# scylladb/vector-store

Measured on NVIDIA B200. Metric: ann_search_qps_at_recall10_ge_0.95, higher is better.
Workload: dtype bf16

## Files before the change

vector-store_b200/csrc/graph_search.cuh:

```cuda
#pragma once
#ifdef VSB_K4B_PROFILE
#include <cstdio>
#endif
#include "kernels.h"
#include "select.cuh"

namespace vsb {

constexpr int K4_WARPS = 4;
constexpr uint32_t kHashEmpty = 0xFFFFFFFFu;

struct K4Args {
    const uint8_t* q_rows;
    const float* q_nrm;
    uint32_t nq, q_row_bytes;
    const uint8_t* x_rows;
    const float* x_nrm;
    uint32_t x_row_bytes;
    const uint32_t* graph;
    uint32_t graph_stride, degree;
    const uint64_t* seed_lists;
    uint32_t seed_splits, n_seeds;
    const uint32_t* seed_slots;
    const uint32_t* deny;
    const uint64_t* keys;
    uint32_t itopk, max_iters, k, hash_bits, search_width, queue_cap;
    int metric;
    uint64_t* out_keys;
    float* out_dists;
    uint32_t* out_counts;
    uint64_t* out_packed;
    long long self_base;
    uint32_t out_stride;
    unsigned long long* counters;
    const uint32_t* allow;
    uint64_t allow_bits;
    uint32_t rk;
    uint32_t mma;
    uint32_t compact;
    uint32_t l2pf;
};

__device__ __forceinline__ bool hash_insert(uint32_t* tab, uint32_t mask, uint32_t bits, uint32_t slot) {
    uint32_t h = (slot * 0x9E3779B1u) >> (32 - bits);
#pragma unroll 1
    for (int probe = 0; probe < 64; ++probe) {
        const uint32_t old = atomicCAS(&tab[h], kHashEmpty, slot);
        if (old == kHashEmpty) return true;
        if (old == slot) return false;
        h = (h + 1) & mask;
    }
    return false;
}

constexpr uint16_t kTagEmpty = 0xFFFFu;
__device__ __forceinline__ bool hash_insert16(uint16_t* tab, uint32_t mask, uint32_t bits, uint32_t slot) {
    uint32_t h = (slot * 0x9E3779B1u) >> (32 - bits);
    uint32_t t = (slot * 0x85EBCA6Bu) >> 16;
    const unsigned short tag = (unsigned short)(t == kTagEmpty ? 0xFFFEu : t);
#pragma unroll 1
    for (int probe = 0; probe < 64; ++probe) {
        const unsigned short old = atomicCAS(reinterpret_cast<unsigned short*>(&tab[h]), (unsigned short)kTagEmpty, tag);
        if (old == kTagEmpty) return true;
        if (old == tag) return false;
        h = (h + 1) & mask;
    }
    return false;
}

template <int CPL, int U>
struct VecGroup {
    uint4 x[U][CPL];
};

template <int CPL, int U>
__device__ __forceinline__ void group_load(VecGroup<CPL, U>& g, const uint8_t* __restrict__ x_rows, uint32_t row_bytes,
                                           const uint32_t* newq, uint32_t base, uint32_t stride, uint32_t last,
                                           int lane, int n_chunks, bool full) {
#pragma unroll
    for (int u = 0; u < U; ++u) {
        uint32_t idx = base + u * stride;
        idx = idx < last ? idx : last;
        const uint4* xrow = reinterpret_cast<const uint4*>(x_rows + (size_t)newq[idx] * row_bytes) + lane;
        if (full) {
#pragma unroll
            for (int j = 0; j < CPL; ++j) g.x[u][j] = ldg_nc_v4(xrow + j * 32);
        } else {
#pragma unroll
            for (int j = 0; j < CPL; ++j) {
                g.x[u][j] = make_uint4(0, 0, 0, 0);
                if (j * 32 + lane < n_chunks) g.x[u][j] = ldg_nc_v4(xrow + j * 32);
            }
        }
    }
}

template <int ST, int CPL, int U>
__device__ __forceinline__ void group_reduce(const VecGroup<CPL, U>& g, const float* qf, const uint4* qc, bool is_l2,
                                             float* newd, uint32_t base, uint32_t stride, uint32_t n_new, int lane) {
    constexpr int E = Storage<ST>::ELEMS;
    constexpr bool kFloat = Storage<ST>::kFloat;
#pragma unroll
    for (int u = 0; u < U; ++u) {
        const uint32_t idx = base + u * stride;
        float raw;
        if constexpr (kFloat) {
            float f;
            if (is_l2) {
                ChunkAcc<ST, VSB_METRIC_L2SQ> acc;
#pragma unroll
                for (int j = 0; j < CPL; ++j) {
                    float xf[E];
                    Storage<ST>::unpack(g.x[u][j], xf);
                    acc.add_f(&qf[j * E], xf);
                }
                f = acc.f;
            } else {
                ChunkAcc<ST, VSB_METRIC_IP> acc;
#pragma unroll
                for (int j = 0; j < CPL; ++j) {
                    float xf[E];
                    Storage<ST>::unpack(g.x[u][j], xf);
                    acc.add_f(&qf[j * E], xf);
                }
                f = acc.f;
            }
            raw = butterfly_sum(f);
        } else {
            int i;
            if (is_l2) {
                ChunkAcc<ST, VSB_METRIC_L2SQ> acc;
#pragma unroll
                for (int j = 0; j < CPL; ++j) acc.add(qc[j], g.x[u][j]);
                i = acc.i;
            } else {
                ChunkAcc<ST, VSB_METRIC_IP> acc;
#pragma unroll
                for (int j = 0; j < CPL; ++j) acc.add(qc[j], g.x[u][j]);
                i = acc.i;
            }
            raw = (float)butterfly_sum_i(i);
        }
        if (lane == 0 && idx < n_new) newd[idx] = raw;
    }
}

template <int ST>
__device__ __forceinline__ float finish_raw(float raw, int metric, float qn, float xn) {
    if constexpr (ST == VSB_ST_B1) {
        return raw;
    } else {
        if (metric == VSB_METRIC_L2SQ) return raw;
        if (metric == VSB_METRIC_IP) {
            if constexpr (ST == VSB_ST_I8) raw = __fdiv_rn(raw, 16129.0f);
            return __fsub_rn(1.0f, raw);
        }
        if (qn == 0.0f && xn == 0.0f) return 0.0f;
        if (qn == 0.0f || xn == 0.0f) return 1.0f;
        float d = __fsub_rn(1.0f, __fdiv_rn(raw, __fmul_rn(qn, xn)));
        d = d < 0.0f ? 0.0f : d;
        d = d > 2.0f ? 2.0f : d;
        return d;
    }
}

template <int ST>
__device__ __forceinline__ void mma_16816(float (&c)[4], uint32_t a0, uint32_t a1, uint32_t a2, uint32_t a3, uint32_t b0,
                                          uint32_t b1) {
    if constexpr (ST == VSB_ST_BF16) {
        asm volatile("mma.sync.aligned.m16n8k16.row.col.f32.bf16.bf16.f32 {%0,%1,%2,%3}, {%4,%5,%6,%7}, {%8,%9}, {%0,%1,%2,%3};"
                     : "+f"(c[0]), "+f"(c[1]), "+f"(c[2]), "+f"(c[3])
                     : "r"(a0), "r"(a1), "r"(a2), "r"(a3), "r"(b0), "r"(b1));
    } else {
        asm volatile("mma.sync.aligned.m16n8k16.row.col.f32.f16.f16.f32 {%0,%1,%2,%3}, {%4,%5,%6,%7}, {%8,%9}, {%0,%1,%2,%3};"
                     : "+f"(c[0]), "+f"(c[1]), "+f"(c[2]), "+f"(c[3])
                     : "r"(a0), "r"(a1), "r"(a2), "r"(a3), "r"(b0), "r"(b1));
    }
}

template <int ST, int CPL, int U>
__device__ __forceinline__ void group_reduce_mma(const VecGroup<CPL, U>& grp, const uint4* qc, float* newd, uint32_t base,
                                                 uint32_t stride, uint32_t n_new, int lane) {
    const int g = lane >> 2, t = lane & 3;
    const bool diag = t == (g >> 1);
    const bool odd = (g & 1) != 0;
#pragma unroll
    for (int u = 0; u < U; u += 2) {
        constexpr bool kPair = U > 1;
        float c[4] = {0.f, 0.f, 0.f, 0.f};
#pragma unroll
        for (int j = 0; j < CPL; ++j) {
            const uint4 xa = grp.x[u][j];
            const uint4 xb = kPair ? grp.x[kPair ? u + 1 : u][j] : xa;
            mma_16816<ST>(c, xa.x, xb.x, xa.y, xb.y, qc[j].x, qc[j].y);
            mma_16816<ST>(c, xa.z, xb.z, xa.w, xb.w, qc[j].z, qc[j].w);
        }
        float v0 = diag ? (odd ? c[1] : c[0]) : 0.0f;
        float v1 = diag ? (odd ? c[3] : c[2]) : 0.0f;
        v0 = butterfly_sum(v0);
        if (kPair) v1 = butterfly_sum(v1);
        if (lane == 0) {
            const uint32_t i0 = base + u * stride, i1 = base + (u + 1) * stride;
            if (i0 < n_new) newd[i0] = v0;
            if (kPair && i1 < n_new) newd[i1] = v1;
        }
    }
}

__device__ __forceinline__ void prefetch_row_l2(const void* p, uint32_t bytes) {
    asm volatile("cp.async.bulk.prefetch.L2.global [%0], %1;" ::"l"(p), "r"(bytes) : "memory");
}

template <int ST, int CPL, int U, bool MMA = false>
__device__ __forceinline__ void evaluate_entries(const uint8_t* __restrict__ x_rows, uint32_t row_bytes,
                                                 const uint32_t* newq, float* newd, uint32_t first, uint32_t stride,
                                                 uint32_t mine, uint32_t n_new, const float* qf, const uint4* qc,
                                                 bool is_l2, int lane, int n_chunks, bool full, uint32_t l2pf = 0) {
    if (mine == 0) return;
    const uint32_t last = first + (mine - 1) * stride;
    if (l2pf != 0) {
        for (uint32_t m = 2 * U + lane; m < l2pf + 2 * U && m < mine; m += 32)
            prefetch_row_l2(x_rows + (size_t)newq[first + m * stride] * row_bytes, row_bytes);
    }
    auto reduce = [&](const VecGroup<CPL, U>& grp, uint32_t base) {
        if constexpr (MMA) group_reduce_mma<ST, CPL, U>(grp, qc, newd, base, stride, n_new, lane);
        else group_reduce<ST, CPL, U>(grp, qf, qc, is_l2, newd, base, stride, n_new, lane);
    };
    VecGroup<CPL, U> ga, gb;
    group_load<CPL, U>(ga, x_rows, row_bytes, newq, first, stride, last, lane, n_chunks, full);
    for (uint32_t m0 = 0; m0 < mine; m0 += 2 * U) {
        const bool has_b = m0 + U < mine;
        if (l2pf != 0) {
            const uint32_t m = m0 + 2 * U + l2pf + lane;
            if (lane < 2 * U && m < mine) prefetch_row_l2(x_rows + (size_t)newq[first + m * stride] * row_bytes, row_bytes);
        }
        if (has_b) group_load<CPL, U>(gb, x_rows, row_bytes, newq, first + (m0 + U) * stride, stride, last, lane, n_chunks, full);
        reduce(ga, first + m0 * stride);
        if (has_b) {
            if (m0 + 2 * U < mine)
                group_load<CPL, U>(ga, x_rows, row_bytes, newq, first + (m0 + 2 * U) * stride, stride, last, lane, n_chunks, full);
            reduce(gb, first + (m0 + U) * stride);
        }
    }
}

#ifndef VSB_K4_MAX_WIDTH
#define VSB_K4_MAX_WIDTH 4
#endif
constexpr int K4_MAX_WIDTH = VSB_K4_MAX_WIDTH;

template <int ST, int CPL, bool MMA = false>
constexpr int k4_min_blocks() { return (ST == VSB_ST_I8 && CPL <= 2) ? 4 : 3; }
template <int CPL, bool MMA>
constexpr int k4_rows_per_group() { return CPL <= 3 ? 4 : (CPL <= 6 ? 2 : 1); }

template <int ST, int CPL, bool FILTER, bool MMA = false>
__global__ void __launch_bounds__(K4_WARPS * 32, k4_min_blocks<ST, CPL, MMA>()) graph_search_kernel(K4Args a) {
    constexpr int E = Storage<ST>::ELEMS;
    constexpr bool kFloat = Storage<ST>::kFloat;
    constexpr int U = k4_rows_per_group<CPL, MMA>();
    constexpr int QF = (kFloat && !MMA) ? CPL * E : 1;

    extern __shared__ __align__(16) uint8_t smem_raw[];
    const int lane = threadIdx.x & 31, warp = threadIdx.x >> 5;
    const uint32_t q = blockIdx.x * K4_WARPS + warp;
    if (q >= a.nq) return;

    const uint32_t hsize = 1u << a.hash_bits, hmask = hsize - 1;
    const uint32_t qcap = a.queue_cap;
    const size_t per_warp = (size_t)a.itopk * 8 + (size_t)hsize * 2 + (size_t)qcap * 8 + (FILTER ? (size_t)a.rk * 8 : 0) + 64 * 8;
    uint64_t* list = reinterpret_cast<uint64_t*>(smem_raw + (size_t)warp * per_warp);
    uint16_t* hash = reinterpret_cast<uint16_t*>(list + a.itopk);
    uint32_t* newq = reinterpret_cast<uint32_t*>(hash + hsize);
    float* newd = reinterpret_cast<float*>(newq + qcap);
    uint64_t* rlist = reinterpret_cast<uint64_t*>(newd + qcap);
    uint64_t* stage = rlist + (FILTER ? a.rk : 0);
    if constexpr (FILTER) {
        for (uint32_t i = lane; i < a.rk; i += 32) rlist[i] = kInvalidPacked;
    }
    const LessBySlot less;
    const bool is_l2 = a.metric == VSB_METRIC_L2SQ;
    const bool is_cos = a.metric == VSB_METRIC_COS;
    const int n_chunks = a.x_row_bytes / 16;
    const bool full = n_chunks == CPL * 32;

    for (uint32_t i = lane; i < a.itopk; i += 32) list[i] = kInvalidPacked;
    for (uint32_t i = lane; i < hsize; i += 32) hash[i] = kTagEmpty;

    const uint4* qrow = reinterpret_cast<const uint4*>(a.q_rows + (size_t)q * a.q_row_bytes);
    float qf[QF];
    uint4 qc[(kFloat && !MMA) ? 1 : CPL];
#pragma unroll
    for (int j = 0; j < CPL; ++j) {
        const int c = j * 32 + lane;
        uint4 v = make_uint4(0, 0, 0, 0);
        if (c < n_chunks) v = qrow[c];
        if constexpr (kFloat && !MMA)
            Storage<ST>::unpack(v, &qf[j * E]);
        else
            qc[j] = v;
    }
    if constexpr (MMA) qf[0] = 0.0f;
    const float qn = a.q_nrm[q];
    __syncwarp();

    uint32_t n_hashed = 0, n_new = 0;
    unsigned long long n_evals = 0, n_parents = 0;

    auto enqueue = [&](uint32_t nb) {
        bool is_new = false;
        if (nb != kInvalidSlot) is_new = hash_insert16(hash, hmask, a.hash_bits, nb);
        const uint32_t m = __ballot_sync(kFullMask, is_new);
        if (is_new) newq[n_new + __popc(m & ((1u << lane) - 1))] = nb;
        n_new += __popc(m);
        n_hashed += __popc(m);
    };

    auto evaluate_queue = [&]() {
        __syncwarp();
        if (n_new == 0) return;
        n_evals += n_new;
        float xn_pre[2] = {0.0f, 0.0f};
        if constexpr (MMA) {
            if (is_cos || is_l2) {
                if (lane < n_new) xn_pre[0] = __ldg(a.x_nrm + newq[lane]);
                if (32 + lane < n_new) xn_pre[1] = __ldg(a.x_nrm + newq[32 + lane]);
            }
        }
        evaluate_entries<ST, CPL, U, MMA>(a.x_rows, a.x_row_bytes, newq, newd, 0, 1, n_new, n_new, qf, qc, is_l2, lane,
                                          n_chunks, full, a.l2pf);
        __syncwarp();
        uint64_t worst = list[a.itopk - 1];
        uint32_t n_stage = 0;
        auto fold_stage = [&](uint32_t n) {
            __syncwarp();
            uint64_t v = lane < n ? stage[lane] : kInvalidPacked;
            v = warp_sort32(v, lane, less);
            warp_list_merge(list, (int)a.itopk, v, lane, less);
            worst = list[a.itopk - 1];
        };
        for (uint32_t base = 0; base < n_new; base += 32) {
            uint64_t res = kInvalidPacked;
            if (base + lane < n_new) {
                const uint32_t slot = newq[base + lane];
                float xn = 0.0f;
                if (MMA && base < 64) xn = base == 0 ? xn_pre[0] : xn_pre[1];
                else if (is_cos || (MMA && is_l2)) xn = __ldg(a.x_nrm + slot);
                float raw = newd[base + lane];
                if constexpr (MMA) {
                    if (is_l2) raw = fmaxf(fmaf(-2.0f, raw, fmaf(qn, qn, xn * xn)), 0.0f);
                }
                res = pack_ds(finish_raw<ST>(raw, a.metric, qn, xn), slot);
            }
            if constexpr (FILTER) {
                uint64_t adm = kInvalidPacked;
                if (res != kInvalidPacked) {
                    const uint64_t row_id = a.keys[packed_lo(res)] & kRowMask48;
                    if (row_id < a.allow_bits && (a.allow[row_id >> 5] >> (row_id & 31) & 1u)) adm = res;
                }
                if (__ballot_sync(kFullMask, adm < rlist[a.rk - 1]) != 0) {
                    adm = warp_sort32(adm, lane, less);
                    warp_list_merge(rlist, (int)a.rk, adm, lane, less);
                }
            }
            const bool keep = res < worst;
            const uint32_t km = __ballot_sync(kFullMask, keep);
            if (km == 0) continue;
            if (!a.compact || n_new <= 32) {
                res = warp_sort32(res, lane, less);
                warp_list_merge(list, (int)a.itopk, res, lane, less);
                continue;
            }
            if (keep) stage[n_stage + __popc(km & ((1u << lane) - 1))] = res;
            n_stage += __popc(km);
            if (n_stage >= 32) {
                fold_stage(32);
                __syncwarp();
                const uint64_t mv = lane + 32 < n_stage ? stage[32 + lane] : kInvalidPacked;
                __syncwarp();
                if (lane + 32 < n_stage) stage[lane] = mv;
                n_stage -= 32;
            }
        }
        if (n_stage != 0) fold_stage(n_stage);
        n_new = 0;
    };

    {
        uint64_t sv = kInvalidPacked;
        for (uint32_t s = 0; s < a.seed_splits; ++s) {
            uint64_t v = a.seed_lists[((size_t)q * a.seed_splits + s) * 32 + lane];
            v = warp_sort32(v, lane, less);
            const uint64_t rc = shfl_u64(v, 31 - lane);
            sv = warp_bitonic_merge32(rc < sv ? rc : sv, lane, less);
        }
        uint32_t nb = kInvalidSlot;
        if (lane < (int)a.n_seeds && sv != kInvalidPacked) nb = a.seed_slots[packed_lo(sv)];
        enqueue(nb);
        evaluate_queue();
    }

    const uint32_t width = a.search_width;
    for (uint32_t it = 0; it < a.max_iters; ++it) {
        if (n_hashed > (hsize >> 2) * 3) {
            for (uint32_t i = lane; i < hsize; i += 32) hash[i] = kTagEmpty;
            __syncwarp();
            n_hashed = 0;
            for (uint32_t b = 0; b < a.itopk; b += 32) {
                const uint64_t e = list[b + lane];
                if (e != kInvalidPacked) hash_insert16(hash, hmask, a.hash_bits, packed_lo(e) & ~kExpandedBit);
                n_hashed += __popc(__ballot_sync(kFullMask, e != kInvalidPacked));
            }
            __syncwarp();
        }
        uint32_t par[K4_MAX_WIDTH];
        uint32_t np = 0;
#pragma unroll
        for (int i = 0; i < K4_MAX_WIDTH; ++i) par[i] = kInvalidSlot;
        for (uint32_t b = 0; b < a.itopk && np < width; b += 32) {
            const uint64_t e = list[b + lane];
            const bool unexp = e != kInvalidPacked && !(packed_lo(e) & kExpandedBit);
            uint32_t m = __ballot_sync(kFullMask, unexp);
            bool mine = false;
            while (m && np < width) {
                const int src = __ffs(m) - 1;
                m &= m - 1;
                const uint32_t pslot = __shfl_sync(kFullMask, packed_lo(e), src);
#pragma unroll
                for (int i = 0; i < K4_MAX_WIDTH; ++i)
                    if (i == (int)np) par[i] = pslot;
                if (lane == src) mine = true;
                ++np;
            }
            if (mine) list[b + lane] = e | kExpandedBit;
        }
        __syncwarp();
        if (np == 0) break;
        n_parents += np;
        uint32_t nbs[K4_MAX_WIDTH][2];
#pragma unroll
        for (int i = 0; i < K4_MAX_WIDTH; ++i) {
#pragma unroll
            for (int h = 0; h < 2; ++h) {
                nbs[i][h] = kInvalidSlot;
                const uint32_t r = h * 32 + lane;
                if (i < (int)np && r < a.degree) nbs[i][h] = __ldg(a.graph + (size_t)par[i] * a.graph_stride + r);
            }
        }
#pragma unroll
        for (int i = 0; i < K4_MAX_WIDTH; ++i) {
#pragma unroll
            for (int h = 0; h < 2; ++h) {
                if (i < (int)np && h * 32 < (int)a.degree) enqueue(nbs[i][h]);
            }
        }
        evaluate_queue();
    }

    __syncwarp();
    const uint64_t* src_list = FILTER ? rlist : list;
    const uint32_t src_len = FILTER ? a.rk : a.itopk;
    uint32_t count = 0;
    for (uint32_t b = 0; b < src_len; b += 32) {
        const uint64_t e = src_list[b + lane];
        const uint32_t slot = packed_lo(e) & ~kExpandedBit;
        bool valid = e != kInvalidPacked;
        if (valid && a.deny != nullptr && bit_test(a.deny, slot)) valid = false;
        if (valid && a.self_base >= 0 && slot == (uint32_t)(a.self_base + q)) valid = false;
        const uint32_t m = __ballot_sync(kFullMask, valid);
        const uint32_t pos = count + __popc(m & ((1u << lane) - 1));
        if (valid && pos < a.k) {
            if (a.out_packed != nullptr) {
                a.out_packed[(size_t)q * a.out_stride + pos] = ((uint64_t)packed_hi(e) << 32) | slot;
            } else {
                a.out_keys[(size_t)q * a.k + pos] = a.keys[slot];
                a.out_dists[(size_t)q * a.k + pos] = ord_to_f32(packed_hi(e));
            }
        }
        count += __popc(m);
    }
    if (count > a.k) count = a.k;
    if (a.out_packed != nullptr) {
        for (uint32_t i = count + lane; i < a.out_stride; i += 32) a.out_packed[(size_t)q * a.out_stride + i] = kInvalidPacked;
    }
    for (uint32_t i = count + lane; i < a.k; i += 32) {
        if (a.out_packed != nullptr) {
        } else {
            a.out_keys[(size_t)q * a.k + i] = 0xFFFFFFFFFFFFFFFFull;
            a.out_dists[(size_t)q * a.k + i] = __int_as_float(0x7F800000);
        }
    }
    if (lane == 0) {
        if (a.out_counts != nullptr) a.out_counts[q] = count;
        if (a.counters != nullptr) {
            atomicAdd(&a.counters[0], n_evals);
            atomicAdd(&a.counters[1], n_parents);
        }
    }
}

constexpr int K4B_WARPS = 8;
constexpr int K4B_MAX_WIDTH = 8;
constexpr int K4B_PICK_ROUNDS = 4;

#ifdef VSB_K4B_PROFILE
#define K4B_T(i)                                       \
    do {                                               \
        const long long now_ = clock64();              \
        prof_[i] += now_ - prof_t_;                    \
        prof_t_ = now_;                                \
    } while (0)
#else
#define K4B_T(i) do { } while (0)
#endif

template <int ST, int CPL>
__global__ void __launch_bounds__(K4B_WARPS * 32, 1) graph_search_cta_kernel(K4Args a) {
    constexpr int E = Storage<ST>::ELEMS;
    constexpr bool kFloat = Storage<ST>::kFloat;
    constexpr int U = CPL <= 3 ? 4 : (CPL <= 6 ? 2 : 1);
    constexpr int QF = kFloat ? CPL * E : 1;

    extern __shared__ __align__(16) uint8_t smem_raw[];
    const int tid = threadIdx.x, lane = tid & 31, warp = tid >> 5;
    const uint32_t q = blockIdx.x;
    const uint32_t hsize = 1u << a.hash_bits, hmask = hsize - 1;
    const uint32_t qcap = a.queue_cap;
    uint64_t* list = reinterpret_cast<uint64_t*>(smem_raw);
    uint64_t* list_alt = list + a.itopk;
    uint64_t* newp = list_alt + a.itopk;
    uint32_t* hash = reinterpret_cast<uint32_t*>(newp + qcap);
    uint32_t* newq = hash + hsize;
    float* newd = reinterpret_cast<float*>(newq + qcap);
    uint32_t* par = reinterpret_cast<uint32_t*>(newd + qcap);
    uint32_t* ctrl = par + K4B_MAX_WIDTH;
    uint32_t* wcnt = ctrl + 4;
    const LessBySlot less;
    const bool is_l2 = a.metric == VSB_METRIC_L2SQ;
    const bool is_cos = a.metric == VSB_METRIC_COS;
    const int n_chunks = a.x_row_bytes / 16;
    const bool full = n_chunks == CPL * 32;

    for (uint32_t i = tid; i < a.itopk; i += K4B_WARPS * 32) list[i] = kInvalidPacked;
    for (uint32_t i = tid; i < hsize; i += K4B_WARPS * 32) hash[i] = kHashEmpty;
    if (tid < 4) ctrl[tid] = 0;

    const uint4* qrow = reinterpret_cast<const uint4*>(a.q_rows + (size_t)q * a.q_row_bytes);
    float qf[QF];
    uint4 qc[kFloat ? 1 : CPL];
#pragma unroll
    for (int j = 0; j < CPL; ++j) {
        const int c = j * 32 + lane;
        uint4 v = make_uint4(0, 0, 0, 0);
        if (c < n_chunks) v = qrow[c];
        if constexpr (kFloat)
            Storage<ST>::unpack(v, &qf[j * E]);
        else
            qc[j] = v;
    }
    const float qn = a.q_nrm[q];
    unsigned long long n_evals = 0, n_parents = 0;
    __syncthreads();
#ifdef VSB_K4B_PROFILE
    long long prof_[8] = {0, 0, 0, 0, 0, 0, 0, 0};
    long long prof_t_ = clock64();
    const long long prof_start_ = prof_t_;
#endif

    const uint32_t width = a.search_width;
    const uint32_t deg_pad = ((a.degree + 31) / 32) * 32;
    auto pick_parents = [&]() {
        uint64_t e[K4B_PICK_ROUNDS];
        uint32_t m[K4B_PICK_ROUNDS];
#pragma unroll
        for (int r = 0; r < K4B_PICK_ROUNDS; ++r) {
            const uint32_t t = r * K4B_WARPS * 32 + tid;
            e[r] = t < a.itopk ? list[t] : kInvalidPacked;
            const bool unexp = e[r] != kInvalidPacked && !(packed_lo(e[r]) & kExpandedBit);
            m[r] = __ballot_sync(kFullMask, unexp);
            if (lane == 0) wcnt[r * K4B_WARPS + warp] = __popc(m[r]);
        }
        __syncthreads();
        uint32_t before = 0, total = 0;
#pragma unroll
        for (int r = 0; r < K4B_PICK_ROUNDS; ++r) {
#pragma unroll
            for (int w = 0; w < K4B_WARPS; ++w) {
                const uint32_t c = wcnt[r * K4B_WARPS + w];
                total += c;
            }
        }
#pragma unroll
        for (int r = 0; r < K4B_PICK_ROUNDS; ++r) {
            uint32_t base = before;
#pragma unroll
            for (int w = 0; w < K4B_WARPS; ++w) {
                const uint32_t c = wcnt[r * K4B_WARPS + w];
                if (w < warp) base += c;
                before += c;
            }
            if (m[r] >> lane & 1u) {
                const uint32_t rank = base + __popc(m[r] & ((1u << lane) - 1));
                if (rank < width) {
                    par[rank] = packed_lo(e[r]);
                    list[r * K4B_WARPS * 32 + tid] = e[r] | kExpandedBit;
                } else if (rank < 2 * width) {
                    asm volatile("prefetch.global.L2 [%0];" ::"l"(a.graph + (size_t)packed_lo(e[r]) * a.graph_stride));
                }
            }
        }
        const uint32_t np = total < width ? total : width;
        if (tid == 0) {
            ctrl[1] = np;
            n_parents += np;
        }
        __syncthreads();
    };

    auto lower_bound = [&](const uint64_t* seq, uint32_t len, uint64_t x) -> uint32_t {
        uint32_t lo = 0, n = len;
        while (n > 0) {
            const uint32_t half = n >> 1;
            const bool go = seq[lo + half] < x;
            lo = go ? lo + half + 1 : lo;
            n = go ? n - half - 1 : half;
        }
        return lo;
    };

    auto evaluate_queue = [&]() {
        K4B_T(0);
        __syncthreads();
        K4B_T(1);
        const uint32_t n_new = ctrl[0];
        if (n_new != 0) {
            const uint32_t mine = n_new > (uint32_t)warp ? (n_new - warp + K4B_WARPS - 1) / K4B_WARPS : 0;
            float xn_first = 0.0f;
            if (is_cos && (uint32_t)tid < n_new) xn_first = __ldg(a.x_nrm + newq[tid]);
            evaluate_entries<ST, CPL, U>(a.x_rows, a.x_row_bytes, newq, newd, (uint32_t)warp, K4B_WARPS, mine, n_new, qf, qc,
                                         is_l2, lane, n_chunks, full);
            K4B_T(2);
            __syncthreads();
            K4B_T(3);
            const uint64_t worst = list[a.itopk - 1];
            for (uint32_t i = tid; i < n_new; i += K4B_WARPS * 32) {
                const uint32_t slot = newq[i];
                const float xn = !is_cos ? 0.0f : (i == (uint32_t)tid ? xn_first : __ldg(a.x_nrm + slot));
                const uint64_t res = pack_ds(finish_raw<ST>(newd[i], a.metric, qn, xn), slot);
                if (res < worst) newp[atomicAdd(&ctrl[3], 1u)] = res;
            }
            for (uint32_t i = tid; i < a.itopk; i += K4B_WARPS * 32) list_alt[i] = kInvalidPacked;
            __syncthreads();
            K4B_T(4);
            const uint32_t n_keep = ctrl[3];
            for (uint32_t g = warp; g * 32 < n_keep; g += K4B_WARPS) {
                const uint64_t res = g * 32 + lane < n_keep ? newp[g * 32 + lane] : kInvalidPacked;
                newp[g * 32 + lane] = warp_sort32(res, lane, less);
            }
            __syncthreads();
            K4B_T(5);
            if (n_keep != 0) {
                const uint32_t n_groups = (n_keep + 31) / 32;
                for (uint32_t i = tid; i < a.itopk + n_groups * 32; i += K4B_WARPS * 32) {
                    const bool from_list = i < a.itopk;
                    const uint32_t own_g = from_list ? 0xFFFFFFFFu : (i - a.itopk) >> 5;
                    const uint64_t x = from_list ? list[i] : newp[i - a.itopk];
                    if (x == kInvalidPacked) continue;
                    uint32_t pos = from_list ? i : ((i - a.itopk) & 31u) + lower_bound(list, a.itopk, x);
                    for (uint32_t g = 0; g < n_groups; ++g)
                        if (g != own_g) pos += lower_bound(newp + g * 32, 32, x);
                    if (pos < a.itopk) list_alt[pos] = x;
                }
                uint64_t* t = list;
                list = list_alt;
                list_alt = t;
            }
            if (tid == 0) {
                ctrl[2] += n_new;
                ctrl[0] = 0;
                ctrl[3] = 0;
                n_evals += n_new;
            }
            __syncthreads();
        }
        K4B_T(6);
        pick_parents();
        K4B_T(7);
    };

    if (warp == 0) {
        uint64_t sv = kInvalidPacked;
        for (uint32_t s = 0; s < a.seed_splits; ++s) {
            uint64_t v = a.seed_lists[((size_t)q * a.seed_splits + s) * 32 + lane];
            v = warp_sort32(v, lane, less);
            const uint64_t rc = shfl_u64(v, 31 - lane);
            sv = warp_bitonic_merge32(rc < sv ? rc : sv, lane, less);
        }
        uint32_t nb = kInvalidSlot;
        if (lane < (int)a.n_seeds && sv != kInvalidPacked) nb = a.seed_slots[packed_lo(sv)];
        bool is_new = false;
        if (nb != kInvalidSlot) is_new = hash_insert(hash, hmask, a.hash_bits, nb);
        const uint32_t m = __ballot_sync(kFullMask, is_new);
        if (is_new) newq[__popc(m & ((1u << lane) - 1))] = nb;
        if (lane == 0) ctrl[0] = __popc(m);
    }
    evaluate_queue();

    for (uint32_t it = 0; it < a.max_iters; ++it) {
        if (ctrl[2] > (hsize >> 2) * 3) {
            __syncthreads();
            for (uint32_t i = tid; i < hsize; i += K4B_WARPS * 32) hash[i] = kHashEmpty;
            __syncthreads();
            uint32_t cnt = 0;
            for (uint32_t i = tid; i < a.itopk; i += K4B_WARPS * 32) {
                const uint64_t e = list[i];
                if (e != kInvalidPacked) {
                    hash_insert(hash, hmask, a.hash_bits, packed_lo(e) & ~kExpandedBit);
                    ++cnt;
                }
            }
            if (tid == 0) ctrl[2] = 0;
            __syncthreads();
            if (cnt) atomicAdd(&ctrl[2], cnt);
            __syncthreads();
        }
        const uint32_t np = ctrl[1];
        if (np == 0) break;
        for (uint32_t t = tid; t < np * deg_pad; t += K4B_WARPS * 32) {
            const uint32_t i = t / deg_pad, r = t % deg_pad;
            if (r < a.degree) {
                const uint32_t nb = __ldg(a.graph + (size_t)par[i] * a.graph_stride + r);
                if (nb != kInvalidSlot && hash_insert(hash, hmask, a.hash_bits, nb)) newq[atomicAdd(&ctrl[0], 1u)] = nb;
            }
        }
        evaluate_queue();
    }

#ifdef VSB_K4B_PROFILE
    if (tid == 0 && q == 0)
        printf("k4b cycles: total %lld | fetch %lld wait %lld | rows %lld wait %lld | finish %lld sort %lld fold %lld pick %lld | "
               "evals %llu parents %llu\n",
               clock64() - prof_start_, prof_[0], prof_[1], prof_[2], prof_[3], prof_[4], prof_[5], prof_[6], prof_[7], n_evals,
               n_parents);
#endif
    if (warp == 0) {
        uint32_t count = 0;
        for (uint32_t b = 0; b < a.itopk; b += 32) {
            const uint64_t e = list[b + lane];
            const uint32_t slot = packed_lo(e) & ~kExpandedBit;
            bool valid = e != kInvalidPacked;
            if (valid && a.deny != nullptr && bit_test(a.deny, slot)) valid = false;
            if (valid && a.self_base >= 0 && slot == (uint32_t)(a.self_base + q)) valid = false;
            const uint32_t m = __ballot_sync(kFullMask, valid);
            const uint32_t pos = count + __popc(m & ((1u << lane) - 1));
            if (valid && pos < a.k) {
                if (a.out_packed != nullptr) {
                    a.out_packed[(size_t)q * a.out_stride + pos] = ((uint64_t)packed_hi(e) << 32) | slot;
                } else {
                    a.out_keys[(size_t)q * a.k + pos] = a.keys[slot];
                    a.out_dists[(size_t)q * a.k + pos] = ord_to_f32(packed_hi(e));
                }
            }
            count += __popc(m);
        }
        if (count > a.k) count = a.k;
        if (a.out_packed != nullptr) {
            for (uint32_t i = count + lane; i < a.out_stride; i += 32) a.out_packed[(size_t)q * a.out_stride + i] = kInvalidPacked;
        }
        for (uint32_t i = count + lane; i < a.k; i += 32) {
            if (a.out_packed != nullptr) {
            } else {
                a.out_keys[(size_t)q * a.k + i] = 0xFFFFFFFFFFFFFFFFull;
                a.out_dists[(size_t)q * a.k + i] = __int_as_float(0x7F800000);
            }
        }
        if (lane == 0) {
            if (a.out_counts != nullptr) a.out_counts[q] = count;
            if (a.counters != nullptr) {
                atomicAdd(&a.counters[0], n_evals);
                atomicAdd(&a.counters[1], n_parents);
            }
        }
    }
}

constexpr int SEED_SCAN_WARPS = 8;
constexpr int SEED_SCAN_ROWS_PER_WARP = 4;

template <int ST>
__global__ void __launch_bounds__(SEED_SCAN_WARPS * 32) seed_scan_kernel(const uint8_t* __restrict__ q_rows,
                                                                          const float* __restrict__ q_nrm,
                                                                          uint32_t q_row_bytes,
                                                                          const uint8_t* __restrict__ s_rows,
                                                                          const float* __restrict__ s_nrm,
                                                                          uint32_t n_seed_rows, uint32_t row_bytes,
                                                                          int metric, uint32_t n_blocks,
                                                                          uint64_t* __restrict__ out) {
    __shared__ uint64_t best[SEED_SCAN_WARPS];
    const int lane = threadIdx.x & 31, warp = threadIdx.x >> 5;
    const uint32_t q = blockIdx.y;
    const uint4* qrow = reinterpret_cast<const uint4*>(q_rows + (size_t)q * q_row_bytes);
    const float qn = q_nrm[q];
    const int n_chunks = row_bytes / 16;
    const uint32_t r0 = (blockIdx.x * SEED_SCAN_WARPS + warp) * SEED_SCAN_ROWS_PER_WARP;
    uint64_t mine = kInvalidPacked;
#pragma unroll
    for (int i = 0; i < SEED_SCAN_ROWS_PER_WARP; ++i) {
        const uint32_t r = r0 + i;
        if (r >= n_seed_rows) break;
        const uint4* xrow = reinterpret_cast<const uint4*>(s_rows + (size_t)r * row_bytes);
        float d;
        if constexpr (ST == VSB_ST_B1) {
            d = warp_distance<ST, VSB_METRIC_HAMMING>(qrow, xrow, n_chunks, qn, 0.0f, lane);
        } else {
            if (metric == VSB_METRIC_L2SQ) d = warp_distance<ST, VSB_METRIC_L2SQ>(qrow, xrow, n_chunks, qn, 0.0f, lane);
            else if (metric == VSB_METRIC_IP) d = warp_distance<ST, VSB_METRIC_IP>(qrow, xrow, n_chunks, qn, 0.0f, lane);
            else d = warp_distance<ST, VSB_METRIC_COS>(qrow, xrow, n_chunks, qn, s_nrm[r], lane);
        }
        const uint64_t p = pack_ds(d, r);
        mine = p < mine ? p : mine;
    }
    if (lane == 0) best[warp] = mine;
    __syncthreads();
    if (threadIdx.x == 0) {
        uint64_t b = best[0];
        for (int w = 1; w < SEED_SCAN_WARPS; ++w) b = best[w] < b ? best[w] : b;
        out[(size_t)q * n_blocks * 32 + blockIdx.x] = b;
    }
}

template <int ST, int CPL>
void launch_k4_inst(const K4Args& a, dim3 grid, size_t smem, cudaStream_t stream) {
    if (a.allow != nullptr) {
        cudaFuncSetAttribute(graph_search_kernel<ST, CPL, true>, cudaFuncAttributeMaxDynamicSharedMemorySize, (int)smem);
        graph_search_kernel<ST, CPL, true><<<grid, K4_WARPS * 32, smem, stream>>>(a);
        return;
    }
    if constexpr (ST == VSB_ST_BF16 || ST == VSB_ST_F16) {
        if (a.mma) {
            cudaFuncSetAttribute(graph_search_kernel<ST, CPL, false, true>, cudaFuncAttributeMaxDynamicSharedMemorySize, (int)smem);
            graph_search_kernel<ST, CPL, false, true><<<grid, K4_WARPS * 32, smem, stream>>>(a);
            return;
        }
    }
    cudaFuncSetAttribute(graph_search_kernel<ST, CPL, false>, cudaFuncAttributeMaxDynamicSharedMemorySize, (int)smem);
    graph_search_kernel<ST, CPL, false><<<grid, K4_WARPS * 32, smem, stream>>>(a);
}

template <int ST, int CPL>
void launch_k4b_inst(const K4Args& a, dim3 grid, size_t smem, cudaStream_t stream) {
    cudaFuncSetAttribute(graph_search_cta_kernel<ST, CPL>, cudaFuncAttributeMaxDynamicSharedMemorySize, (int)smem);
    graph_search_cta_kernel<ST, CPL><<<grid, K4B_WARPS * 32, smem, stream>>>(a);
}

template <int ST>
void launch_k4b_storage(const K4Args& a, int cpl, dim3 grid, size_t smem, cudaStream_t stream) {
    switch (cpl) {
        case 1: launch_k4b_inst<ST, 1>(a, grid, smem, stream); break;
        case 2: launch_k4b_inst<ST, 2>(a, grid, smem, stream); break;
        case 3: launch_k4b_inst<ST, 3>(a, grid, smem, stream); break;
        case 4: launch_k4b_inst<ST, 4>(a, grid, smem, stream); break;
        case 6: launch_k4b_inst<ST, 6>(a, grid, smem, stream); break;
        case 8: launch_k4b_inst<ST, 8>(a, grid, smem, stream); break;
        default: launch_k4b_inst<ST, 12>(a, grid, smem, stream); break;
    }
}

struct SeedScanArgs {
    const uint8_t* q_rows; const float* q_nrm; uint32_t nq, q_row_bytes;
    const uint8_t* s_rows; const float* s_nrm; uint32_t n_seed_rows, row_bytes;
    int metric; uint32_t n_blocks; uint64_t* out;
};
template <int ST>
void launch_seed_scan_storage(const SeedScanArgs& s, cudaStream_t stream) {
    const uint32_t ctas = (s.n_seed_rows + SEED_SCAN_WARPS * SEED_SCAN_ROWS_PER_WARP - 1) /
                          (SEED_SCAN_WARPS * SEED_SCAN_ROWS_PER_WARP);
    seed_scan_kernel<ST><<<dim3(ctas, s.nq), SEED_SCAN_WARPS * 32, 0, stream>>>(
        s.q_rows, s.q_nrm, s.q_row_bytes, s.s_rows, s.s_nrm, s.n_seed_rows, s.row_bytes, s.metric, s.n_blocks, s.out);
}

template <int ST>
void launch_k4_storage(const K4Args& a, int cpl, dim3 grid, size_t smem, cudaStream_t stream) {
    switch (cpl) {
        case 1: launch_k4_inst<ST, 1>(a, grid, smem, stream); break;
        case 2: launch_k4_inst<ST, 2>(a, grid, smem, stream); break;
        case 3: launch_k4_inst<ST, 3>(a, grid, smem, stream); break;
        case 4: launch_k4_inst<ST, 4>(a, grid, smem, stream); break;
        case 6: launch_k4_inst<ST, 6>(a, grid, smem, stream); break;
        case 8: launch_k4_inst<ST, 8>(a, grid, smem, stream); break;
        default: launch_k4_inst<ST, 12>(a, grid, smem, stream); break;
    }
}

#define VSB_K4_DECL(name)                                                                              \
    void launch_k4b_##name(const K4Args& a, int cpl, dim3 grid, size_t smem, cudaStream_t stream);     \
    void launch_seed_scan_##name(const SeedScanArgs& s, cudaStream_t stream);
VSB_K4_DECL(f32)
VSB_K4_DECL(f16)
VSB_K4_DECL(bf16)
VSB_K4_DECL(i8)
VSB_K4_DECL(b1)
void launch_k4_f32(const K4Args& a, int cpl, dim3 grid, size_t smem, cudaStream_t stream);
void launch_k4_f16(const K4Args& a, int cpl, dim3 grid, size_t smem, cudaStream_t stream);
void launch_k4_bf16(const K4Args& a, int cpl, dim3 grid, size_t smem, cudaStream_t stream);
void launch_k4_i8(const K4Args& a, int cpl, dim3 grid, size_t smem, cudaStream_t stream);
void launch_k4_b1(const K4Args& a, int cpl, dim3 grid, size_t smem, cudaStream_t stream);

}
```

Measured before the change: 1.188 million.

## Split graph search into query warps and MMA distance-eval warps via smem ring

Replaces the per-warp MMA graph search with a warp-specialized CTA. Twelve query warps run traversal and hashing, then publish row chunks into a shared-memory ring guarded by mbarriers. Eight evaluation warps, given more registers through setmaxnreg, pull chunks and compute tensor-core distances. The aim is to overlap traversal bookkeeping with distance computation and raise load throughput, at the cost of cross-warp synchronisation overhead, one CTA per SM, and query warps spinning while they wait for their distances.

```diff
diff --git a/vector-store_b200/csrc/graph_search.cuh b/vector-store_b200/csrc/graph_search.cuh
--- a/vector-store_b200/csrc/graph_search.cuh
+++ b/vector-store_b200/csrc/graph_search.cuh
@@ -39,6 +39,7 @@
     uint32_t mma;
     uint32_t compact;
     uint32_t l2pf;
+    uint32_t queries_per_cta;
 };
 
 __device__ __forceinline__ bool hash_insert(uint32_t* tab, uint32_t mask, uint32_t bits, uint32_t slot) {
@@ -211,7 +212,7 @@
     asm volatile("cp.async.bulk.prefetch.L2.global [%0], %1;" ::"l"(p), "r"(bytes) : "memory");
 }
 
-template <int ST, int CPL, int U, bool MMA = false>
+template <int ST, int CPL, int U>
 __device__ __forceinline__ void evaluate_entries(const uint8_t* __restrict__ x_rows, uint32_t row_bytes,
                                                  const uint32_t* newq, float* newd, uint32_t first, uint32_t stride,
                                                  uint32_t mine, uint32_t n_new, const float* qf, const uint4* qc,
@@ -223,8 +224,7 @@
             prefetch_row_l2(x_rows + (size_t)newq[first + m * stride] * row_bytes, row_bytes);
     }
     auto reduce = [&](const VecGroup<CPL, U>& grp, uint32_t base) {
-        if constexpr (MMA) group_reduce_mma<ST, CPL, U>(grp, qc, newd, base, stride, n_new, lane);
-        else group_reduce<ST, CPL, U>(grp, qf, qc, is_l2, newd, base, stride, n_new, lane);
+        group_reduce<ST, CPL, U>(grp, qf, qc, is_l2, newd, base, stride, n_new, lane);
     };
     VecGroup<CPL, U> ga, gb;
     group_load<CPL, U>(ga, x_rows, row_bytes, newq, first, stride, last, lane, n_chunks, full);
@@ -249,27 +249,21 @@
 #endif
 constexpr int K4_MAX_WIDTH = VSB_K4_MAX_WIDTH;
 
-template <int ST, int CPL, bool MMA = false>
+template <int ST, int CPL>
 constexpr int k4_min_blocks() { return (ST == VSB_ST_I8 && CPL <= 2) ? 4 : 3; }
-template <int CPL, bool MMA>
+template <int CPL>
 constexpr int k4_rows_per_group() { return CPL <= 3 ? 4 : (CPL <= 6 ? 2 : 1); }
 
-template <int ST, int CPL, bool FILTER, bool MMA = false>
-__global__ void __launch_bounds__(K4_WARPS * 32, k4_min_blocks<ST, CPL, MMA>()) graph_search_kernel(K4Args a) {
-    constexpr int E = Storage<ST>::ELEMS;
-    constexpr bool kFloat = Storage<ST>::kFloat;
-    constexpr int U = k4_rows_per_group<CPL, MMA>();
-    constexpr int QF = (kFloat && !MMA) ? CPL * E : 1;
-
-    extern __shared__ __align__(16) uint8_t smem_raw[];
-    const int lane = threadIdx.x & 31, warp = threadIdx.x >> 5;
-    const uint32_t q = blockIdx.x * K4_WARPS + warp;
-    if (q >= a.nq) return;
-
+__host__ __device__ inline size_t k4_query_bytes(uint32_t itopk, uint32_t hash_bits, uint32_t queue_cap, uint32_t rk) {
+    return (size_t)itopk * 8 + ((size_t)2 << hash_bits) + (size_t)queue_cap * 8 + (size_t)rk * 8 + 64 * 8;
+}
+
+template <int ST, bool FILTER, bool MMA, class Evaluate>
+__device__ __forceinline__ void k4_search_query(const K4Args& a, uint32_t q, uint8_t* blk, int lane, float qn,
+                                                Evaluate&& evaluate) {
     const uint32_t hsize = 1u << a.hash_bits, hmask = hsize - 1;
     const uint32_t qcap = a.queue_cap;
-    const size_t per_warp = (size_t)a.itopk * 8 + (size_t)hsize * 2 + (size_t)qcap * 8 + (FILTER ? (size_t)a.rk * 8 : 0) + 64 * 8;
-    uint64_t* list = reinterpret_cast<uint64_t*>(smem_raw + (size_t)warp * per_warp);
+    uint64_t* list = reinterpret_cast<uint64_t*>(blk);
     uint16_t* hash = reinterpret_cast<uint16_t*>(list + a.itopk);
     uint32_t* newq = reinterpret_cast<uint32_t*>(hash + hsize);
     float* newd = reinterpret_cast<float*>(newq + qcap);
@@ -281,27 +275,9 @@
     const LessBySlot less;
     const bool is_l2 = a.metric == VSB_METRIC_L2SQ;
     const bool is_cos = a.metric == VSB_METRIC_COS;
-    const int n_chunks = a.x_row_bytes / 16;
-    const bool full = n_chunks == CPL * 32;
 
     for (uint32_t i = lane; i < a.itopk; i += 32) list[i] = kInvalidPacked;
     for (uint32_t i = lane; i < hsize; i += 32) hash[i] = kTagEmpty;
-
-    const uint4* qrow = reinterpret_cast<const uint4*>(a.q_rows + (size_t)q * a.q_row_bytes);
-    float qf[QF];
-    uint4 qc[(kFloat && !MMA) ? 1 : CPL];
-#pragma unroll
-    for (int j = 0; j < CPL; ++j) {
-        const int c = j * 32 + lane;
-        uint4 v = make_uint4(0, 0, 0, 0);
-        if (c < n_chunks) v = qrow[c];
-        if constexpr (kFloat && !MMA)
-            Storage<ST>::unpack(v, &qf[j * E]);
-        else
-            qc[j] = v;
-    }
-    if constexpr (MMA) qf[0] = 0.0f;
-    const float qn = a.q_nrm[q];
     __syncwarp();
 
     uint32_t n_hashed = 0, n_new = 0;
@@ -320,15 +296,8 @@
         __syncwarp();
         if (n_new == 0) return;
         n_evals += n_new;
-        float xn_pre[2] = {0.0f, 0.0f};
-        if constexpr (MMA) {
-            if (is_cos || is_l2) {
-                if (lane < n_new) xn_pre[0] = __ldg(a.x_nrm + newq[lane]);
-                if (32 + lane < n_new) xn_pre[1] = __ldg(a.x_nrm + newq[32 + lane]);
-            }
-        }
-        evaluate_entries<ST, CPL, U, MMA>(a.x_rows, a.x_row_bytes, newq, newd, 0, 1, n_new, n_new, qf, qc, is_l2, lane,
-                                          n_chunks, full, a.l2pf);
+        float xn_pre[K4_MAX_WIDTH];
+        evaluate(static_cast<const uint32_t*>(newq), newd, n_new, xn_pre);
         __syncwarp();
         uint64_t worst = list[a.itopk - 1];
         uint32_t n_stage = 0;
@@ -344,8 +313,13 @@
             if (base + lane < n_new) {
                 const uint32_t slot = newq[base + lane];
                 float xn = 0.0f;
-                if (MMA && base < 64) xn = base == 0 ? xn_pre[0] : xn_pre[1];
-                else if (is_cos || (MMA && is_l2)) xn = __ldg(a.x_nrm + slot);
+                if (MMA && base < 32 * K4_MAX_WIDTH) {
+#pragma unroll
+                    for (int i = 0; i < K4_MAX_WIDTH; ++i)
+                        if (base == 32u * i) xn = xn_pre[i];
+                } else if (is_cos || (MMA && is_l2)) {
+                    xn = __ldg(a.x_nrm + slot);
+                }
                 float raw = newd[base + lane];
                 if constexpr (MMA) {
                     if (is_l2) raw = fmaxf(fmaf(-2.0f, raw, fmaf(qn, qn, xn * xn)), 0.0f);
@@ -496,6 +470,258 @@
             atomicAdd(&a.counters[0], n_evals);
             atomicAdd(&a.counters[1], n_parents);
         }
+    }
+}
+
+template <int ST, int CPL, bool FILTER>
+__global__ void __launch_bounds__(K4_WARPS * 32, k4_min_blocks<ST, CPL>()) graph_search_kernel(K4Args a) {
+    constexpr int E = Storage<ST>::ELEMS;
+    constexpr bool kFloat = Storage<ST>::kFloat;
+    constexpr int U = k4_rows_per_group<CPL>();
+    constexpr int QF = kFloat ? CPL * E : 1;
+
+    extern __shared__ __align__(16) uint8_t smem_raw[];
+    const int lane = threadIdx.x & 31, warp = threadIdx.x >> 5;
+    const uint32_t q = blockIdx.x * K4_WARPS + warp;
+    if (q >= a.nq) return;
+    const size_t per_warp = k4_query_bytes(a.itopk, a.hash_bits, a.queue_cap, FILTER ? a.rk : 0);
+    const bool is_l2 = a.metric == VSB_METRIC_L2SQ;
+    const int n_chunks = a.x_row_bytes / 16;
+    const bool full = n_chunks == CPL * 32;
+
+    const uint4* qrow = reinterpret_cast<const uint4*>(a.q_rows + (size_t)q * a.q_row_bytes);
+    float qf[QF];
+    uint4 qc[kFloat ? 1 : CPL];
+#pragma unroll
+    for (int j = 0; j < CPL; ++j) {
+        const int c = j * 32 + lane;
+        uint4 v = make_uint4(0, 0, 0, 0);
+        if (c < n_chunks) v = qrow[c];
+        if constexpr (kFloat)
+            Storage<ST>::unpack(v, &qf[j * E]);
+        else
+            qc[j] = v;
+    }
+    k4_search_query<ST, FILTER, false>(a, q, smem_raw + (size_t)warp * per_warp, lane, a.q_nrm[q],
+                                       [&](const uint32_t* newq, float* newd, uint32_t n_new, float*) {
+                                           evaluate_entries<ST, CPL, U>(a.x_rows, a.x_row_bytes, newq, newd, 0, 1, n_new,
+                                                                        n_new, qf, qc, is_l2, lane, n_chunks, full, a.l2pf);
+                                       });
+}
+
+constexpr int K4S_QUERY_WARPS = 12, K4S_EVAL_WARPS = 8;
+constexpr int K4S_LAUNCH_REGS = 96, K4S_QUERY_REGS = 72, K4S_EVAL_REGS = 128;
+static_assert(K4S_QUERY_WARPS % 4 == 0 && K4S_EVAL_WARPS % 4 == 0, "roles are whole warpgroups (setmaxnreg)");
+static_assert((K4S_QUERY_WARPS + K4S_EVAL_WARPS) * 32 * K4S_LAUNCH_REGS <= 65536, "launch exceeds the register file");
+static_assert(K4S_QUERY_WARPS * K4S_QUERY_REGS + K4S_EVAL_WARPS * K4S_EVAL_REGS <=
+                  (K4S_QUERY_WARPS + K4S_EVAL_WARPS) * K4S_LAUNCH_REGS,
+              "register split exceeds the registers the CTA is launched with");
+constexpr uint32_t K4S_EXIT = 0xFFu;
+
+__host__ __device__ inline size_t k4s_query_bytes(uint32_t itopk, uint32_t hash_bits, uint32_t queue_cap, int cpl) {
+    return k4_query_bytes(itopk, hash_bits, queue_cap, 0) + (size_t)cpl * 512 + 16;
+}
+__host__ __device__ inline uint32_t k4s_chunks_per_query(uint32_t queue_cap, int u) { return (queue_cap + u - 1) / u; }
+__host__ __device__ inline uint32_t k4s_ring_slots(uint32_t qpc, uint32_t queue_cap, int u) {
+    return qpc * k4s_chunks_per_query(queue_cap, u) + K4S_EVAL_WARPS;
+}
+__host__ __device__ inline size_t k4s_smem_bytes(uint32_t qpc, uint32_t itopk, uint32_t hash_bits, uint32_t queue_cap, int cpl,
+                                                 int u) {
+    return (size_t)qpc * k4s_query_bytes(itopk, hash_bits, queue_cap, cpl) + (size_t)k4s_ring_slots(qpc, queue_cap, u) * 24 + 16;
+}
+
+__device__ __forceinline__ uint32_t smem_addr(const void* p) { return (uint32_t)__cvta_generic_to_shared(p); }
+__device__ __forceinline__ void mbar_init(uint64_t* b, uint32_t count) {
+    asm volatile("mbarrier.init.shared::cta.b64 [%0], %1;" ::"r"(smem_addr(b)), "r"(count) : "memory");
+}
+__device__ __forceinline__ void mbar_arrive(uint64_t* b, uint32_t count) {
+    asm volatile("{\n.reg .b64 st;\nmbarrier.arrive.release.cta.shared::cta.b64 st, [%0], %1;\n}" ::"r"(smem_addr(b)), "r"(count)
+                 : "memory");
+}
+__device__ __forceinline__ bool mbar_try_wait(uint64_t* b, uint32_t parity) {
+    uint32_t ok;
+    asm volatile("{\n.reg .pred p;\nmbarrier.try_wait.parity.acquire.cta.shared::cta.b64 p, [%1], %2;\nselp.u32 %0, 1, 0, p;\n}"
+                 : "=r"(ok)
+                 : "r"(smem_addr(b)), "r"(parity)
+                 : "memory");
+    return ok != 0;
+}
+__device__ __forceinline__ uint64_t ld_acquire_shared(const uint64_t* p) {
+    uint64_t v;
+    asm volatile("ld.acquire.cta.shared::cta.u64 %0, [%1];" : "=l"(v) : "r"(smem_addr(p)) : "memory");
+    return v;
+}
+__device__ __forceinline__ void st_release_shared(uint64_t* p, uint64_t v) {
+    asm volatile("st.release.cta.shared::cta.u64 [%0], %1;" ::"r"(smem_addr(p)), "l"(v) : "memory");
+}
+
+struct K4sRing {
+    uint64_t* word;
+    uint64_t* full;
+    uint64_t* empty;
+    uint32_t* ctr;
+    uint32_t n_slots;
+
+    __device__ __forceinline__ void put(uint32_t pos, uint32_t payload) const {
+        const uint32_t s = pos % n_slots;
+        while ((uint32_t)(ld_acquire_shared(word + s) >> 32) != pos) mbar_try_wait(empty + s, ((pos / n_slots) & 1u) ^ 1u);
+        st_release_shared(word + s, ((uint64_t)(pos + 1) << 32) | payload);
+        mbar_arrive(full + s, 1);
+    }
+    __device__ __forceinline__ uint32_t take(uint32_t pos, int lane) const {
+        const uint32_t s = pos % n_slots;
+        uint64_t w;
+        while ((uint32_t)((w = ld_acquire_shared(word + s)) >> 32) != pos + 1) mbar_try_wait(full + s, (pos / n_slots) & 1u);
+        __syncwarp();
+        if (lane == 0) {
+            st_release_shared(word + s, (uint64_t)(pos + n_slots) << 32);
+            mbar_arrive(empty + s, 1);
+        }
+        return (uint32_t)w;
+    }
+    template <class Payload>
+    __device__ __forceinline__ void publish(uint32_t n, int lane, Payload&& payload) const {
+        uint32_t t0 = 0;
+        if (lane == 0) t0 = atomicAdd(&ctr[1], n);
+        t0 = __shfl_sync(kFullMask, t0, 0);
+        for (uint32_t i = lane; i < n; i += 32) put(t0 + i, payload(i));
+        __syncwarp();
+    }
+};
+
+template <int ST, int CPL>
+__global__ void __launch_bounds__((K4S_QUERY_WARPS + K4S_EVAL_WARPS) * 32, 1) graph_search_split_kernel(K4Args a) {
+    constexpr int U = k4_rows_per_group<CPL>();
+    extern __shared__ __align__(16) uint8_t smem_raw[];
+    const int lane = threadIdx.x & 31, warp = threadIdx.x >> 5;
+    const uint32_t qpc = a.queries_per_cta;
+    const size_t per_q = k4s_query_bytes(a.itopk, a.hash_bits, a.queue_cap, CPL);
+    const size_t blk_bytes = k4_query_bytes(a.itopk, a.hash_bits, a.queue_cap, 0);
+    const uint32_t cap1 = k4s_chunks_per_query(a.queue_cap, U) + 1;
+    K4sRing ring;
+    ring.n_slots = k4s_ring_slots(qpc, a.queue_cap, U);
+    ring.word = reinterpret_cast<uint64_t*>(smem_raw + qpc * per_q);
+    ring.full = ring.word + ring.n_slots;
+    ring.empty = ring.full + ring.n_slots;
+    ring.ctr = reinterpret_cast<uint32_t*>(ring.empty + ring.n_slots);
+    auto qrow_of = [&](uint32_t w) { return reinterpret_cast<uint4*>(smem_raw + w * per_q + blk_bytes); };
+    auto qbar_of = [&](uint32_t w) { return reinterpret_cast<uint64_t*>(smem_raw + w * per_q + blk_bytes + CPL * 512); };
+
+    for (uint32_t i = threadIdx.x; i < ring.n_slots; i += blockDim.x) {
+        ring.word[i] = (uint64_t)i << 32;
+        mbar_init(ring.full + i, 1);
+        mbar_init(ring.empty + i, 1);
+    }
+    if (threadIdx.x < qpc) mbar_init(qbar_of(threadIdx.x), cap1);
+    if (threadIdx.x < 3) ring.ctr[threadIdx.x] = 0;
+    __syncthreads();
+
+    if (warp < K4S_QUERY_WARPS) {
+        asm volatile("setmaxnreg.dec.sync.aligned.u32 %0;" ::"n"(K4S_QUERY_REGS));
+        const uint32_t w = (uint32_t)warp;
+        const uint32_t q = blockIdx.x * qpc + w;
+        if (w < qpc && q < a.nq) {
+            const int n_chunks = a.x_row_bytes / 16;
+            const bool is_l2 = a.metric == VSB_METRIC_L2SQ;
+            const bool is_cos = a.metric == VSB_METRIC_COS;
+            const uint4* qsrc = reinterpret_cast<const uint4*>(a.q_rows + (size_t)q * a.q_row_bytes);
+            uint4* qrow = qrow_of(w);
+            for (int c = lane; c < CPL * 32; c += 32) qrow[c] = c < n_chunks ? qsrc[c] : make_uint4(0, 0, 0, 0);
+            uint64_t* qbar = qbar_of(w);
+            uint32_t phase = 0;
+            k4_search_query<ST, false, true>(
+                a, q, smem_raw + w * per_q, lane, a.q_nrm[q],
+                [&](const uint32_t* newq, float*, uint32_t n_new, float* xn) {
+                    const uint32_t n_ch = (n_new + U - 1) / U;
+                    ring.publish(n_ch, lane, [&](uint32_t c) {
+                        const uint32_t first = c * U;
+                        const uint32_t cnt = n_new - first < (uint32_t)U ? n_new - first : (uint32_t)U;
+                        return w | first << 8 | cnt << 24;
+                    });
+                    if (lane == 0) mbar_arrive(qbar, cap1 - n_ch);
+#pragma unroll
+                    for (int i = 0; i < K4_MAX_WIDTH; ++i) {
+                        xn[i] = 0.0f;
+                        if ((is_cos || is_l2) && i * 32 + lane < (int)n_new) xn[i] = __ldg(a.x_nrm + newq[i * 32 + lane]);
+                    }
+                    while (!mbar_try_wait(qbar, phase)) {
+                    }
+                    phase ^= 1u;
+                });
+        }
+        __syncwarp();
+        if (lane == 0 && atomicAdd(&ring.ctr[2], 1u) == K4S_QUERY_WARPS - 1) {
+            for (uint32_t t = atomicAdd(&ring.ctr[1], K4S_EVAL_WARPS), i = 0; i < K4S_EVAL_WARPS; ++i) ring.put(t + i, K4S_EXIT);
+        }
+        return;
+    }
+
+    asm volatile("setmaxnreg.inc.sync.aligned.u32 %0;" ::"n"(K4S_EVAL_REGS));
+    const int n_chunks = a.x_row_bytes / 16;
+    const bool full = n_chunks == CPL * 32;
+    auto take_next = [&]() -> uint32_t {
+        uint32_t pos = 0;
+        if (lane == 0) pos = atomicAdd(&ring.ctr[0], 1u);
+        return ring.take(__shfl_sync(kFullMask, pos, 0), lane);
+    };
+    auto try_take = [&](uint32_t& payload) -> bool {
+        uint32_t pos = 0xFFFFFFFFu;
+        if (lane == 0) {
+            volatile uint32_t* vc = ring.ctr;
+            uint32_t h = vc[0];
+            while (h < vc[1]) {
+                const uint32_t old = atomicCAS(&ring.ctr[0], h, h + 1);
+                if (old == h) {
+                    pos = h;
+                    break;
+                }
+                h = old;
+            }
+        }
+        pos = __shfl_sync(kFullMask, pos, 0);
+        if (pos == 0xFFFFFFFFu) return false;
+        payload = ring.take(pos, lane);
+        return true;
+    };
+    auto newq_of = [&](uint32_t w) {
+        return reinterpret_cast<const uint32_t*>(smem_raw + w * per_q + (size_t)a.itopk * 8 + ((size_t)2 << a.hash_bits));
+    };
+    auto load = [&](VecGroup<CPL, U>& g, uint32_t p) {
+        const uint32_t w = p & 0xFFu, first = (p >> 8) & 0xFFFFu, cnt = p >> 24;
+        group_load<CPL, U>(g, a.x_rows, a.x_row_bytes, newq_of(w), first, 1, first + cnt - 1, lane, n_chunks, full);
+    };
+    auto reduce = [&](const VecGroup<CPL, U>& g, uint32_t p) {
+        const uint32_t w = p & 0xFFu, first = (p >> 8) & 0xFFFFu, cnt = p >> 24;
+        uint4 qc[CPL];
+        const uint4* qrow = qrow_of(w);
+#pragma unroll
+        for (int j = 0; j < CPL; ++j) qc[j] = qrow[j * 32 + lane];
+        float* newd = const_cast<float*>(reinterpret_cast<const float*>(newq_of(w) + a.queue_cap));
+        group_reduce_mma<ST, CPL, U>(g, qc, newd, first, 1, first + cnt, lane);
+        __syncwarp();
+        if (lane == 0) mbar_arrive(qbar_of(w), 1);
+    };
+    VecGroup<CPL, U> ga, gb;
+    uint32_t pa = take_next(), pb = 0;
+    if ((pa & 0xFFu) == K4S_EXIT) return;
+    load(ga, pa);
+    while (true) {
+        bool more = try_take(pb);
+        if (more && (pb & 0xFFu) != K4S_EXIT) load(gb, pb);
+        reduce(ga, pa);
+        if (!more) {
+            pb = take_next();
+            if ((pb & 0xFFu) != K4S_EXIT) load(gb, pb);
+        }
+        if ((pb & 0xFFu) == K4S_EXIT) return;
+        more = try_take(pa);
+        if (more && (pa & 0xFFu) != K4S_EXIT) load(ga, pa);
+        reduce(gb, pb);
+        if (!more) {
+            pa = take_next();
+            if ((pa & 0xFFu) != K4S_EXIT) load(ga, pa);
+        }
+        if ((pa & 0xFFu) == K4S_EXIT) return;
     }
 }
 
@@ -838,8 +1064,22 @@
     }
     if constexpr (ST == VSB_ST_BF16 || ST == VSB_ST_F16) {
         if (a.mma) {
-            cudaFuncSetAttribute(graph_search_kernel<ST, CPL, false, true>, cudaFuncAttributeMaxDynamicSharedMemorySize, (int)smem);
-            graph_search_kernel<ST, CPL, false, true><<<grid, K4_WARPS * 32, smem, stream>>>(a);
+            static const int smem_max = [] {
+                int dev = 0, v = 0;
+                cudaGetDevice(&dev);
+                cudaDeviceGetAttribute(&v, cudaDevAttrMaxSharedMemoryPerBlockOptin, dev);
+                return v;
+            }();
+            constexpr int U = k4_rows_per_group<CPL>();
+            K4Args s = a;
+            s.queries_per_cta = K4S_QUERY_WARPS;
+            while (s.queries_per_cta > 1 &&
+                   k4s_smem_bytes(s.queries_per_cta, s.itopk, s.hash_bits, s.queue_cap, CPL, U) > (size_t)smem_max)
+                --s.queries_per_cta;
+            const size_t smem_s = k4s_smem_bytes(s.queries_per_cta, s.itopk, s.hash_bits, s.queue_cap, CPL, U);
+            cudaFuncSetAttribute(graph_search_split_kernel<ST, CPL>, cudaFuncAttributeMaxDynamicSharedMemorySize, (int)smem_s);
+            graph_search_split_kernel<ST, CPL><<<(s.nq + s.queries_per_cta - 1) / s.queries_per_cta,
+                                                 (K4S_QUERY_WARPS + K4S_EVAL_WARPS) * 32, smem_s, stream>>>(s);
             return;
         }
     }
```

Result: slower. 721,700, median of 6 (-39.2%).
